# Happy-ZZX/PL-VIWO

Hardware: NVIDIA B200
Metric: front-end frames/sec @1280x560 (higher is better)
Workload: dtype u8/int32 fixed-point + f32 (LK), f64 (sub-pixel, undistort, RANSAC)

## Files before the change

### pl-viwo_b200/csrc/fe_kernels.h

```cpp
#pragma once
#include <cuda_runtime.h>
#include <atomic>
#include <cstdint>

namespace plviwo {

struct SmemOptIn {
  std::atomic<size_t> granted[64];
  SmemOptIn() { for (auto &g : granted) g.store(0); }
  template <class Kernel>
  void ensure(Kernel kernel, size_t bytes) {
    if (bytes <= 48 * 1024) return;
    int dev = 0;
    cudaGetDevice(&dev);
    std::atomic<size_t> &g = granted[dev & 63];
    if (bytes > g.load(std::memory_order_relaxed)) {
      cudaFuncSetAttribute(kernel, cudaFuncAttributeMaxDynamicSharedMemorySize, (int)bytes);
      g.store(bytes, std::memory_order_relaxed);
    }
  }
};

int carveout_percent();
struct CarveoutOnce {
  std::atomic<bool> done[64];
  CarveoutOnce() { for (auto &d : done) d.store(false); }
  template <class Kernel>
  void apply(Kernel kernel) {
    const int pct = carveout_percent();
    if (pct < 0) return;
    int dev = 0;
    cudaGetDevice(&dev);
    std::atomic<bool> &d = done[dev & 63];
    if (d.load(std::memory_order_relaxed)) return;
    cudaFuncSetAttribute(kernel, cudaFuncAttributePreferredSharedMemoryCarveout, pct);
    d.store(true, std::memory_order_relaxed);
  }
};
#define PLVIWO_CARVEOUT(kernel)   \
  do {                            \
    static CarveoutOnce c__;      \
    c__.apply(kernel);            \
  } while (0)

struct DevImage {
  uint8_t *p = nullptr;
  int w = 0, h = 0, pitch = 0;
};

constexpr int kMaxLevels = 8;
constexpr int kFastBandRows = 16;
constexpr int kMaxWin = 31;

struct Pyramid {
  DevImage lvl[kMaxLevels];
  int n = 0;
};

void launch_hist(const DevImage &src, unsigned *d_hist, cudaStream_t s);
void launch_eq_pyr1(const DevImage &src, unsigned *d_hist, unsigned *d_counter, int equalize, const DevImage &l0,
                    const DevImage &l1, const DevImage &half, cudaStream_t s, const uint8_t *d_clahe_luts = nullptr);
void launch_clahe_lut(const DevImage &src, uint8_t *d_luts, cudaStream_t s);
void launch_pyr_rest(const Pyramid &pyr, unsigned *d_counter, cudaStream_t s);
void launch_pyr_down(const DevImage &src, const DevImage &dst, cudaStream_t s);

void launch_signal(int *host_flag, int value, cudaStream_t s);
void launch_signal_inc(int *host_flag, int *dev_seq, cudaStream_t s);
void init_fld_constants();
void init_device_constants();

struct FastCell {
  int x, y, w, h;
};
void launch_fast(const DevImage &img, const FastCell *d_cells, int n_cells, int max_bands, int max_cell_w, int threshold,
                 unsigned *d_total, int *d_band_off, int *d_band_cnt, unsigned *d_kps, int kps_cap, cudaStream_t s);

void launch_fast_select(const FastCell *d_cells, int n_cells, int max_bands, unsigned *d_total, const int *d_band_off,
                        const int *d_band_cnt, const unsigned *d_kps, int kps_cap, unsigned *d_scratch, int nfg,
                        float2 *d_cand_sel, int *d_cand_cnt, cudaStream_t s);
void host_sort_corners(unsigned *v, int n, int keep = 0);

void launch_corner_subpix(const DevImage &img, const float2 *d_in, float2 *d_out, int n, cudaStream_t s,
                          const int *d_cnt = nullptr, int stride = 0);

struct LkParams {
  int win;
  int max_level;
  int max_count;
  float eps_sq;
  float min_eig;
  double K[4], D[4];
  int undistort;
};
bool launch_lk(const Pyramid &prev, const Pyramid &next, const float2 *d_pts0, float2 *d_pts1, uint8_t *d_status,
               float2 *d_p0n, float2 *d_p1n, int n, const LkParams &prm, cudaStream_t s, int *host_flag = nullptr,
               int flag_value = 0, unsigned *d_done_counter = nullptr, const int *d_tab_cnt = nullptr, int tab_stride = 0,
               bool flow_is_zero = false, const unsigned *cell_mask = nullptr);
bool lk_table_mode_ok(const LkParams &prm, int pyramid_images);
void launch_undistort(const float2 *d_pts, float2 *d_out, int n, const double K[4], const double D[4], cudaStream_t s);

struct FldBuffers {
  unsigned *edges = nullptr;
  int words_per_row = 0;
  int *label = nullptr;
  int *cnt = nullptr;
  int *bbox = nullptr;
  int *lroots = nullptr;
  int *lroot_n = nullptr;
  int lroot_cap = 0;
  int *comp_root = nullptr;
  int *counters = nullptr;
  int2 *chain_pts = nullptr;
  int *chain_seed = nullptr, *chain_off = nullptr, *chain_len = nullptr, *order = nullptr;
  int max_chains = 0;
  float4 *segs = nullptr;
  int *seg_cnt = nullptr;
  float4 *out = nullptr;
  int out_cap = 0;
  int alloc(int w, int h, int length_threshold, int out_capacity);
  void release();
};
constexpr int kMaxLineBatch = 8;
struct FldBatch {
  int n = 0;
  DevImage half[kMaxLineBatch];
  FldBuffers f[kMaxLineBatch];
  __host__ __device__ const DevImage &half_of(int k) const { return half[k]; }
  __host__ __device__ const FldBuffers &fld_of(int k) const { return f[k]; }
};
void launch_canny_batch(const FldBatch &b, float th_low, float th_high, cudaStream_t s);
void launch_fld_batch(const FldBatch &b, int length_threshold, float distance_threshold, cudaStream_t s, cudaEvent_t *ev = nullptr);
constexpr int kSegsPerChainDiv = 21;
void launch_canny(const DevImage &half, float th_low, float th_high, FldBuffers &fb, cudaStream_t s);
void launch_fld(const DevImage &half, int length_threshold, float distance_threshold, FldBuffers &fb, cudaStream_t s,
                cudaEvent_t *ev = nullptr);
void launch_unpack_edges(const FldBuffers &fb, int w, int h, uint8_t *d_out, cudaStream_t s);

struct SlotRec {
  DevImage raw;
  DevImage lvl[kMaxLevels];
  int n_lvl;
  DevImage half;
  uint8_t *mask;
  unsigned *hist, *counters;
  uint8_t *clahe;
  unsigned *fast_total;
  unsigned *kps, *sort_scratch;
  int *band_off, *band_cnt;
  float2 *cand, *cand_ref;
  int *cand_cnt;
  FldBuffers fld;
};
struct FrontJob {
  const uint8_t *src;
  int src_pitch;
  int slot;
  int eq_mode;
  int flags;
};
struct FrontGeom {
  int w, h;
  int n_cells, max_bands, max_cell_w, fast_threshold, kps_cap, nfg;
  const FastCell *cells;
};
void launch_hist_batch(const SlotRec *slots, const FrontJob *jobs, int n_jobs, const FrontGeom &g, int *slot_flags, cudaStream_t s);
void launch_clahe_lut_batch(const SlotRec *slots, const FrontJob *jobs, int n_jobs, const FrontGeom &g, cudaStream_t s);
void launch_eq_pyr1_batch(const SlotRec *slots, const FrontJob *jobs, int n_jobs, const FrontGeom &g, bool want_half, cudaStream_t s);
void launch_pyr_level_batch(const SlotRec *slots, const FrontJob *jobs, int n_jobs, int level, int dw, int dh, cudaStream_t s);
void launch_fast_batch(const SlotRec *slots, const FrontJob *jobs, int n_jobs, const FrontGeom &g, cudaStream_t s);
void launch_fast_select_batch(const SlotRec *slots, const FrontJob *jobs, int n_jobs, const FrontGeom &g, cudaStream_t s);
void launch_corner_subpix_batch(const SlotRec *slots, const FrontJob *jobs, int n_jobs, const FrontGeom &g, cudaStream_t s);
struct FldTable {
  const SlotRec *slots;
  const int *idx;
  __device__ const DevImage &half_of(int k) const { return slots[idx[k]].half; }
  __device__ const FldBuffers &fld_of(int k) const { return slots[idx[k]].fld; }
};
void launch_canny_table(const SlotRec *slots, const int *line_slots, int n_jobs, int w, int h, float th_low, cudaStream_t s);
void launch_fld_table(const SlotRec *slots, const int *line_slots, int n_jobs, int w, int h, int max_chains, int length_threshold,
                      float distance_threshold, cudaStream_t s, cudaEvent_t *ev = nullptr);

}
```

### pl-viwo_b200/csrc/kernels_lines.cu

```cuda
#include "fe_kernels.h"

#include <cstdlib>

#include <algorithm>
#include <mutex>
#include <cstdio>
#include <cmath>

namespace plviwo {

__global__ void k_unpack_edges(const unsigned *__restrict__ edges, int words_per_row, int w, int h,
                               uint8_t *__restrict__ out) {
  int x = blockIdx.x * blockDim.x + threadIdx.x, y = blockIdx.y;
  if (x < w && y < h) out[(size_t)y * w + x] = ((edges[(size_t)y * words_per_row + (x >> 5)] >> (x & 31)) & 1u) ? 255 : 0;
}
void launch_unpack_edges(const FldBuffers &fb, int w, int h, uint8_t *d_out, cudaStream_t s) {
  dim3 grid((w + 255) / 256, h);
  PLVIWO_CARVEOUT(k_unpack_edges);
  k_unpack_edges<<<grid, 256, 0, s>>>(fb.edges, fb.words_per_row, w, h, d_out);
}

__device__ __forceinline__ int ccl_find(const int *parent, int i) {
  int p = __ldcg(parent + i);
  while (p != i) {
// ... 155 lines not shown
  const FldBuffers &fb = b.fld_of(blockIdx.z);
  const unsigned *__restrict__ edges = fb.edges;
  const int words_per_row = fb.words_per_row;
  __shared__ CclTileSmem sm;
  const int tid = threadIdx.x;
  const int x0 = blockIdx.x * kTileW, y0 = blockIdx.y * kTileH;
  if (tid < kTileH * 2) {
    const int r = tid >> 1, k = tid & 1;
    const int gy = y0 + r, gw = (x0 >> 5) + k;
    unsigned v = 0;
    if (gy < h && gw < words_per_row) v = edges[(size_t)gy * words_per_row + gw];
    if (gy < h && (gw << 5) + 32 > w) v &= (gw << 5) < w ? (0xffffffffu >> (32 - (w - (gw << 5)))) : 0u;
    sm.bits[r][k] = v;
  }
  __syncthreads();
  ccl_tile_body(fb, sm, x0, y0, w, h);
}

template <class B>
__global__ void k_ccl_reset(const __grid_constant__ B b) {
  const FldBuffers &fb = b.fld_of(blockIdx.x);
  if (threadIdx.x < 12) fb.counters[threadIdx.x] = 0;
  if (threadIdx.x == 12) *fb.lroot_n = 0;
}

constexpr int kCnW = 64, kCnH = 16, kCnThreads = 256;

static_assert(kCnW == kTileW && kCnH == kTileH && kCnThreads == kTileThreads, "Canny tile = connected-component tile");
struct CannySmem {
  uint8_t pix[kCnH + 4][kCnW + 4];
  short sdx[kCnH + 2][kCnW + 2];
  short sdy[kCnH + 2][kCnW + 2];
  unsigned short mag[kCnH + 2][kCnW + 2];
};
template <class B, bool kFuse>
__global__ void __launch_bounds__(kCnThreads)
    k_canny(const __grid_constant__ B b, int low) {
  const uint8_t *__restrict__ img = b.half_of(blockIdx.z).p;
  const int w = b.half_of(blockIdx.z).w, h = b.half_of(blockIdx.z).h, pitch = b.half_of(blockIdx.z).pitch;
  unsigned *__restrict__ edges = b.fld_of(blockIdx.z).edges;
  const int words_per_row = b.fld_of(blockIdx.z).words_per_row;
  __shared__ __align__(16) uint8_t smem_raw[kFuse ? (sizeof(CclTileSmem) > sizeof(CannySmem) ? sizeof(CclTileSmem) : sizeof(CannySmem))
                                                  : sizeof(CannySmem)];
  __shared__ unsigned s_bits[kCnH][2];
  CannySmem &cs = *reinterpret_cast<CannySmem *>(smem_raw);
  auto &pix = cs.pix;
  auto &sdx = cs.sdx;
  auto &sdy = cs.sdy;
  auto &mag = cs.mag;
  const int tx0 = blockIdx.x * kCnW, ty0 = blockIdx.y * kCnH;
  const int tid = threadIdx.x;
  for (int i = tid; i < (kCnH + 4) * (kCnW + 4); i += kCnThreads) {
    int r = i / (kCnW + 4), c = i - r * (kCnW + 4);
    int gx = min(max(tx0 - 2 + c, 0), w - 1), gy = min(max(ty0 - 2 + r, 0), h - 1);
    pix[r][c] = img[(size_t)gy * pitch + gx];
  }
  __syncthreads();
  for (int i = tid; i < (kCnH + 2) * (kCnW + 2); i += kCnThreads) {
    int r = i / (kCnW + 2), c = i - r * (kCnW + 2);
    int gx = tx0 - 1 + c, gy = ty0 - 1 + r;
    int dx = 0, dy = 0, m = 0;
    if (gx >= 0 && gx < w && gy >= 0 && gy < h) {
      const uint8_t *p = &pix[r + 1][c + 1];
      const int s = kCnW + 4;
      dx = (p[-s + 1] + 2 * p[1] + p[s + 1]) - (p[-s - 1] + 2 * p[-1] + p[s - 1]);
      dy = (p[s - 1] + 2 * p[s] + p[s + 1]) - (p[-s - 1] + 2 * p[-s] + p[-s + 1]);
      m = abs(dx) + abs(dy);
    }
    sdx[r][c] = (short)dx;
    sdy[r][c] = (short)dy;
    mag[r][c] = (unsigned short)m;
  }
  __syncthreads();
  const int wv = tid >> 5, lane = tid & 31;
#pragma unroll
  for (int q = 0; q < 4; q++) {
    int r = 2 * wv + (q >> 1), c = (q & 1) * 32 + lane;
    int gx = tx0 + c, gy = ty0 + r;
    bool edge = false;
    if (gx < w && gy < h) {
      int m = mag[r + 1][c + 1];
      if (m > low) {
        int dx = sdx[r + 1][c + 1], dy = sdy[r + 1][c + 1];
        int x = abs(dx), y = abs(dy) << 15;
        int tg22x = x * 13573;
        if (y < tg22x) {
          edge = m > mag[r + 1][c] && m >= mag[r + 1][c + 2];
        } else {
          int tg67x = tg22x + (x << 16);
          if (y > tg67x) {
            edge = m > mag[r][c + 1] && m >= mag[r + 2][c + 1];
          } else {
            int s = (dx ^ dy) < 0 ? -1 : 1;
            edge = m > mag[r][c + 1 - s] && m > mag[r + 2][c + 1 + s];
          }
        }
      }
      if (gy < 6 && gx < 6) edge = false;
      if (gy >= h - 5 && gx >= w - 5) edge = false;
    }
    unsigned bits = __ballot_sync(0xffffffffu, edge);
    if (lane == 0 && gy < h && (tx0 + (q & 1) * 32) < w) edges[(size_t)gy * words_per_row + ((tx0 + (q & 1) * 32) >> 5)] = bits;
    if (kFuse && lane == 0) s_bits[r][q & 1] = bits;
  }
  if (kFuse) {
    __syncthreads();
    CclTileSmem &ts = *reinterpret_cast<CclTileSmem *>(smem_raw);
    if (tid < kCnH * 2) ts.bits[tid >> 1][tid & 1] = s_bits[tid >> 1][tid & 1];
    __syncthreads();
    ccl_tile_body(b.fld_of(blockIdx.z), ts, tx0, ty0, w, h);
  }
}

template <class B>
static void launch_canny_any(const B &b, int n, int w, int h, float th_low, cudaStream_t s, bool fuse_labels = false) {
  dim3 grid((w + kCnW - 1) / kCnW, (h + kCnH - 1) / kCnH, n);
  if (fuse_labels) {
    PLVIWO_CARVEOUT(k_ccl_reset<B>);
    k_ccl_reset<B><<<n, 32, 0, s>>>(b);
    PLVIWO_CARVEOUT((k_canny<B, true>));
    k_canny<B, true><<<grid, kCnThreads, 0, s>>>(b, (int)floorf(th_low));
    return;
  }
  PLVIWO_CARVEOUT((k_canny<B, false>));
  k_canny<B, false><<<grid, kCnThreads, 0, s>>>(b, (int)floorf(th_low));
}
void launch_canny_batch(const FldBatch &b, float th_low, float th_high, cudaStream_t s) {
  (void)th_high;
  launch_canny_any(b, b.n, b.half[0].w, b.half[0].h, th_low, s);
}
void launch_canny_table(const SlotRec *slots, const int *line_slots, int n_jobs, int w, int h, float th_low, cudaStream_t s) {
  if (n_jobs <= 0) return;
  launch_canny_any(FldTable{slots, line_slots}, n_jobs, w, h, th_low, s, true);
}
void launch_canny(const DevImage &half, float th_low, float th_high, FldBuffers &fb, cudaStream_t s) {
  FldBatch b;
  b.n = 1;
  b.half[0] = half;
  b.f[0] = fb;
  launch_canny_batch(b, th_low, th_high, s);
}

template <class B>
__global__ void k_ccl_border(const __grid_constant__ B b, int w, int h) {
  const FldBuffers &fb = b.fld_of(blockIdx.y);
  const unsigned *__restrict__ edges = fb.edges;
  const int words_per_row = fb.words_per_row;
  int *__restrict__ label = fb.label;
  const int nrow = (h - 1) / kTileH, ncol = (w - 1) / kTileW;
  const int t = blockIdx.x * blockDim.x + threadIdx.x;
  if (t < nrow * w) {
    const int y = (t / w + 1) * kTileH, x = t % w;
    if (!edge_at(edges, words_per_row, x, y)) return;
    const int i = y * w + x;
    if (x > 0 && edge_at(edges, words_per_row, x - 1, y - 1)) ccl_union(label, i, i - w - 1);
    if (edge_at(edges, words_per_row, x, y - 1)) ccl_union(label, i, i - w);
    if (x < w - 1 && edge_at(edges, words_per_row, x + 1, y - 1)) ccl_union(label, i, i - w + 1);
    return;
  }
  const int u = t - nrow * w;
  if (u >= ncol * h) return;
  const int x = (u / h + 1) * kTileW, y = u % h;
  if (!edge_at(edges, words_per_row, x, y)) return;
  const int i = y * w + x;
  if (y > 0 && edge_at(edges, words_per_row, x - 1, y - 1)) ccl_union(label, i, i - w - 1);
  if (edge_at(edges, words_per_row, x - 1, y)) ccl_union(label, i, i - 1);
  if (y < h - 1 && edge_at(edges, words_per_row, x - 1, y + 1)) ccl_union(label, i, i + w - 1);
}

template <class B>
__global__ void k_ccl_link(const __grid_constant__ B b, int w, int h) {
  const FldBuffers &fb = b.fld_of(blockIdx.y);
  int *__restrict__ label = fb.label, *__restrict__ cnt = fb.cnt, *__restrict__ bbox = fb.bbox;
  const int nl = min(*fb.lroot_n, fb.lroot_cap);
  const int n = w * h;
  for (int t = blockIdx.x * blockDim.x + threadIdx.x; t < nl; t += gridDim.x * blockDim.x) {
    const int i = fb.lroots[t];
    const int root = ccl_find(label, i);
    if (root == i) continue;
    atomicExch(label + i, root);
    atomicAdd(cnt + root, cnt[i]);
    atomicMax(bbox + root, bbox[i]);
    atomicMin(bbox + n + root, bbox[n + i]);
    atomicMax(bbox + 2 * n + root, bbox[2 * n + i]);
  }
}

constexpr int kPadRows = 2;
constexpr int kWalkThreads = 128;
constexpr int kWalkWarps = kWalkThreads / 32;
constexpr int kSliceWords = 1600;
constexpr int kTMaxW = 62, kTMaxH = 44;
constexpr int kTRows = kTMaxH + 2;
constexpr int kTLanes = 64;
__host__ __device__ inline int comp_cap_big(int n) { return n / 128 + 1; }

template <class B>
__global__ void k_ccl_roots(const __grid_constant__ B b, int w, int h, int min_pixels, int thread_class) {
  const FldBuffers &fb = b.fld_of(blockIdx.y);
  const int *__restrict__ label = fb.label, *__restrict__ cnt = fb.cnt, *__restrict__ bbox = fb.bbox;
  int *__restrict__ comp_root = fb.comp_root, *__restrict__ counters = fb.counters;
  const int max_comps = fb.max_chains;
  const int nl = min(*fb.lroot_n, fb.lroot_cap);
  const int n = w * h;
  for (int t = blockIdx.x * blockDim.x + threadIdx.x; t < nl; t += gridDim.x * blockDim.x) {
    const int i = fb.lroots[t];
    if (label[i] != i) continue;
    const int c = cnt[i];
    if (c < min_pixels) continue;
    const int bh = bbox[i] - i / w + 1;
    const int groups = (bbox[2 * n + i] >> 5) - (bbox[n + i] >> 5) + 1;
    const int bw = bbox[2 * n + i] - bbox[n + i] + 1;
    if (thread_class && bw <= kTMaxW && bh <= kTMaxH) {
      const int q = atomicAdd(counters + 6, 1);
      if (q < max_comps) comp_root[comp_cap_big(n) + max_comps + q] = i;
    } else if ((bh + 2 * kPadRows) * (groups + 2) > kSliceWords) {
      const int q = atomicAdd(counters + 0, 1);
      if (q < comp_cap_big(n)) comp_root[q] = i;
    } else {
      const int q = atomicAdd(counters + 5, 1);
      if (q < max_comps) comp_root[comp_cap_big(n) + q] = i;
    }
  }
}

static int choose_neighbour_host(unsigned mask, int direction) {
  const int i0 = direction < 0 ? direction + 8 : direction;
  if ((mask >> i0) & 1u) return i0;
  const int ia = (i0 + 1) & 7, ib = (i0 + 7) & 7;
  const bool sa = (mask >> ia) & 1u, sb = (mask >> ib) & 1u;
  if (sa && sb) return ia > ib ? ia : ib;
  if (sa) return ia;
  if (sb) return ib;
  return 8;
}
static inline int nb_dr(int i) { return (i <= 2) ? 1 : ((i == 3 || i == 7) ? 0 : -1); }
static inline int nb_dc(int i) { return (i == 0 || i == 6 || i == 7) ? 1 : ((i == 1 || i == 5) ? 0 : -1); }

constexpr int kKeys = 256;
constexpr int kLut1 = 2 * kKeys * 8;
constexpr int kLut2 = 8 * 8 * 8;
constexpr int kLutSize = kLut1 + kLut2;
__device__ __align__(16) uint8_t g_walk_lut[kLutSize];
static bool g_walk_lut_ready[64] = {false};

void init_fld_constants() {
  static std::mutex mu;
  std::lock_guard<std::mutex> lk(mu);
  int dev = 0;
  cudaGetDevice(&dev);
  if (g_walk_lut_ready[dev & 63]) return;
  static uint8_t lut[kLutSize];
  static const int key_bit[8] = {7, 6, 5, 3, 0, 1, 2, 4};
  for (int first = 0; first < 2; first++)
    for (unsigned key = 0; key < (unsigned)kKeys; key++) {
      unsigned mask = 0;
      for (int i = 0; i < 8; i++) mask |= ((key >> key_bit[i]) & 1u) << i;
      for (int d = 0; d < 8; d++) {
        int i = 8;
        if (mask) i = first ? __builtin_ffs((int)mask) - 1 : choose_neighbour_host(mask, d - 3);
        const int dr = i < 8 ? nb_dr(i) : 0, dc = i < 8 ? nb_dc(i) : 0;
        lut[(first * kKeys + key) * 8 + d] = (uint8_t)(i | ((dr + 1) << 4) | ((dc + 1) << 6));
      }
    }
  for (int sc = 0; sc < 8; sc++)
    for (int d = 0; d < 8; d++)
      for (int i = 0; i < 8; i++) {
        const int cd = i > 4 ? i - 8 : i;
        const int nd = sc == 0 ? cd : ((d - 3) * sc + cd) / (sc + 1);
        lut[kLut1 + (sc * 8 + d) * 8 + i] = (uint8_t)(nd + 3);
      }
  cudaMemcpyToSymbol(g_walk_lut, lut, sizeof(lut));
  g_walk_lut_ready[dev & 63] = true;
}

__device__ __forceinline__ unsigned lds_u32(unsigned addr) {
  unsigned v;
  asm volatile("ld.shared.u32 %0, [%1];" : "=r"(v) : "r"(addr) : "memory");
  return v;
}
__device__ __forceinline__ unsigned lds_u8(unsigned addr) {
  unsigned v;
  asm volatile("ld.shared.u8 %0, [%1];" : "=r"(v) : "r"(addr) : "memory");
  return v;
}
__device__ __forceinline__ uint2 lds_u64(unsigned addr) {
  uint2 v;
  asm volatile("ld.shared.v2.u32 {%0, %1}, [%2];" : "=r"(v.x), "=r"(v.y) : "r"(addr) : "memory");
  return v;
}
__device__ __forceinline__ void sts_u32(unsigned addr, unsigned v) {
  asm volatile("st.shared.u32 [%0], %1;" ::"r"(addr), "r"(v) : "memory");
}

struct WalkCtx {
  const unsigned *edges;
  int words_per_row;
  const int *label, *cnt, *bbox;
  int *counters;
  int2 *chain_pts;
  int *chain_seed, *chain_off, *chain_len;
  int max_chains, w, n, length_threshold;
  bool vec4;
};

__device__ __forceinline__ void walk_gather(const WalkCtx &c, unsigned *bm, int root, int y0, int g0, int groups, int bh, int ws,
                                            int wi, int nw, int lane) {
  const int segs = (groups + 3) >> 2;
  const int items = bh * segs;
  const unsigned gmask = 0xffu << (lane & 24);
  for (int it0 = wi * 4; it0 < items; it0 += nw * 4) {
    int4 lab[4];
    unsigned nib[4];
#pragma unroll
    for (int u = 0; u < 4; u++) {
      const int it = it0 + u;
      nib[u] = 0;
      lab[u] = make_int4(-2, -2, -2, -2);
      if (it < items) {
        const int ly = it / segs, sg = it - ly * segs;
        const int g = 4 * sg + (lane >> 3);
        if (g < groups) {
          const unsigned e = __ldg(c.edges + (size_t)(y0 + ly) * c.words_per_row + g0 + g);
          nib[u] = (e >> (4 * (lane & 7))) & 15u;
          if (nib[u]) {
            const int *lp = c.label + (size_t)(y0 + ly) * c.w + ((g0 + g) << 5) + 4 * (lane & 7);
            if (c.vec4) {
              lab[u] = *reinterpret_cast<const int4 *>(lp);
            } else {
              if (nib[u] & 1u) lab[u].x = lp[0];
              if (nib[u] & 2u) lab[u].y = lp[1];
              if (nib[u] & 4u) lab[u].z = lp[2];
              if (nib[u] & 8u) lab[u].w = lp[3];
            }
          }
        }
      }
    }
#pragma unroll
    for (int u = 0; u < 4; u++) {
      const int it = it0 + u;
      const int l4[4] = {lab[u].x, lab[u].y, lab[u].z, lab[u].w};
      unsigned bits = 0;
#pragma unroll
      for (int k = 0; k < 4; k++) {
        if (!((nib[u] >> k) & 1u)) continue;
        int l = l4[k];
        if (l != root) l = __ldg(c.label + l);
        bits |= (l == root ? 1u : 0u) << k;
      }
      bits = (bits & nib[u]) << (4 * (lane & 7));
      const unsigned word = __reduce_or_sync(gmask, bits);
      if ((lane & 7) == 0 && word && it < items) {
        const int ly = it / segs, sg = it - ly * segs;
        bm[(ly + kPadRows) * ws + 1 + 4 * sg + (lane >> 3)] = word;
      }
    }
  }
}

__device__ __forceinline__ void walk_component(const WalkCtx &c, unsigned *bm, unsigned lut_addr, int root, int y0, int g0, int groups,
                                               int bh, int ws, int lane) {
  const int my_dr = lane < 25 ? lane / 5 - 2 : 0;
  const int my_dc = lane < 25 ? lane % 5 - 2 : 0;
  int npts = 0;
  if (lane == 0) npts = atomicAdd(c.counters + 2, c.cnt[root]);
  npts = __shfl_sync(0xffffffffu, npts, 0);
  const int xbase = (g0 << 5) - 32;
  const unsigned bm_addr = (unsigned)__cvta_generic_to_shared(bm);
  const int my_off = my_dr * ws;
  int sy = 0, sg = 0;
  while (sy < bh) {
    const int g = sg + lane;
    const unsigned v = g < groups ? bm[(sy + kPadRows) * ws + 1 + g] : 0u;
    const unsigned any = __ballot_sync(0xffffffffu, v != 0);
    __syncwarp();
    if (!any) {
      sg += 32;
      if (sg >= groups) { sg = 0; sy++; }
      continue;
    }
    const int first = __ffs(any) - 1;
    const unsigned wv = __shfl_sync(0xffffffffu, v, first);
    sg += first;
    int p = ((sg + 1) << 5) + __ffs(wv) - 1, cy = sy;
    int rb = (cy + kPadRows) * ws;
    const int start = npts;
    const int seed = (y0 + cy) * c.w + xbase + p;
    int step = 0;
    unsigned dsel = 0, sh = 6;
    unsigned tb = lut_addr + kKeys * 8;
    if (lane == 0) sts_u32(bm_addr + 4u * (unsigned)(rb + (p >> 5)), wv & ~(1u << (p & 31)));
    __syncwarp();
    unsigned Bw;
    {
      const int qb = p + my_dc;
      const unsigned word = lds_u32(bm_addr + 4u * (unsigned)(rb + my_off + (qb >> 5)));
      Bw = __ballot_sync(0xffffffffu, (word >> (qb & 31)) & 1u);
      __syncwarp();
    }
    while (true) {
      const int qb = p + my_dc;
      const unsigned waddr = bm_addr + 4u * (unsigned)(rb + my_off + (qb >> 5));
      const unsigned word = lds_u32(waddr);
      const unsigned Bs = Bw >> sh;
      const unsigned key = (Bs & 7u) | ((Bs >> 2) & 8u) | ((Bs >> 3) & 16u) | ((Bs >> 5) & 0xE0u);
      const uint2 ev = lds_u64(tb + key * 8u);
      if (lane == 0) c.chain_pts[npts] = make_int2(xbase + p, y0 + cy);
      npts++;
      Bw = __ballot_sync(0xffffffffu, (word >> (qb & 31)) & 1u);
      __syncwarp();
      const unsigned e = __byte_perm(ev.x, ev.y, dsel);
      const unsigned i = e & 15u;
      if (i == 8u) break;
      dsel = lds_u8(lut_addr + kLut1 + ((unsigned)min(step, 7) * 8u + dsel) * 8u + i);
      step++;
      tb = lut_addr;
      const unsigned r1 = (e >> 4) & 3u, c1 = (e >> 6) & 3u;
      sh = 5u * r1 + c1;
      if (lane == (int)(sh + 6u)) sts_u32(waddr, word & ~(1u << (qb & 31)));
      __syncwarp();
      p += (int)c1 - 1;
      cy += (int)r1 - 1;
      rb += ((int)r1 - 1) * ws;
    }
    if (npts - start < c.length_threshold + 1) {
      npts = start;
    } else if (lane == 0) {
      const int k = atomicAdd(c.counters + 3, 1);
      if (k < c.max_chains) {
        c.chain_seed[k] = seed;
        c.chain_off[k] = start;
        c.chain_len[k] = npts - start;
      }
    }
  }
}

__device__ __forceinline__ void walk_component_single(const WalkCtx &c, unsigned *bm, const uint8_t *lut, int root, int y0, int g0,
                                                      int groups, int bh, int ws) {
  int npts = atomicAdd(c.counters + 2, c.cnt[root]);
  const int xbase = (g0 << 5) - 32;
  int sy = 0, sg = 0;
  while (sy < bh) {
    const int rbs = (sy + kPadRows) * ws;
    unsigned wv = 0;
    while (sg < groups && (wv = bm[rbs + 1 + sg]) == 0u) sg++;
    if (sg >= groups) {
      sg = 0;
      sy++;
      continue;
    }
    int p = ((sg + 1) << 5) + __ffs((int)wv) - 1, cy = sy;
    int rb = rbs;
    const int start = npts;
    const int seed = (y0 + cy) * c.w + xbase + p;
    int step = 0;
    unsigned dsel = 0;
    const uint8_t *tb = lut + kKeys * 8;
    bm[rb + (p >> 5)] = wv & ~(1u << (p & 31));
    while (true) {
      c.chain_pts[npts++] = make_int2(xbase + p, y0 + cy);
      const int q = p - 1, wi = q >> 5, sh = q & 31;
      const unsigned *r0 = bm + rb + wi;
      const unsigned t3 = __funnelshift_r(r0[-ws], r0[-ws + 1], sh) & 7u;
      const unsigned c3 = __funnelshift_r(r0[0], r0[1], sh) & 7u;
      const unsigned b3 = __funnelshift_r(r0[ws], r0[ws + 1], sh) & 7u;
      const unsigned key = t3 | ((c3 & 1u) << 3) | ((c3 >> 2) << 4) | (b3 << 5);
      const unsigned e = tb[key * 8u + dsel];
      const unsigned i = e & 15u;
      if (i == 8u) break;
      dsel = lut[kLut1 + ((unsigned)min(step, 7) * 8u + dsel) * 8u + i];
      step++;
      tb = lut;
      const int dr = (int)((e >> 4) & 3u) - 1, dc = (int)((e >> 6) & 3u) - 1;
      p += dc;
      cy += dr;
      rb += dr * ws;
      bm[rb + (p >> 5)] &= ~(1u << (p & 31));
    }
    if (npts - start < c.length_threshold + 1) {
      npts = start;
    } else {
      const int k = atomicAdd(c.counters + 3, 1);
      if (k < c.max_chains) {
        c.chain_seed[k] = seed;
        c.chain_off[k] = start;
        c.chain_len[k] = npts - start;
      }
    }
  }
}

template <class B>
__global__ void __launch_bounds__(kWalkThreads)
    k_fld_walk_cc(const __grid_constant__ B b, int w, int h, int length_threshold, int coop) {
  const FldBuffers &fb = b.fld_of(blockIdx.y);
  WalkCtx c;
  c.edges = fb.edges;
  c.words_per_row = fb.words_per_row;
  c.label = fb.label;
  c.cnt = fb.cnt;
  c.bbox = fb.bbox;
  c.counters = fb.counters;
  c.chain_pts = fb.chain_pts;
  c.chain_seed = fb.chain_seed;
  c.chain_off = fb.chain_off;
  c.chain_len = fb.chain_len;
  c.max_chains = fb.max_chains;
  c.w = w;
  c.n = w * h;
  c.length_threshold = length_threshold;
  c.vec4 = (w & 3) == 0;
  const int *__restrict__ comp_root = fb.comp_root;
  extern __shared__ __align__(16) uint8_t walk_smem[];
  uint8_t *lut = walk_smem;
  unsigned *arena = reinterpret_cast<unsigned *>(walk_smem + kLutSize);
  __shared__ int s_ci;
  const int tid = threadIdx.x, lane = tid & 31, warp = tid >> 5;
  const int n = c.n;
  const int nBig = min(c.counters[0], comp_cap_big(n));
  const int nSmall = min(c.counters[5], c.max_chains);
  if ((int)blockIdx.x >= nBig && (int)blockIdx.x * kWalkWarps >= nSmall) return;
  for (int i = tid; i < kLutSize / 4; i += kWalkThreads)
    reinterpret_cast<unsigned *>(lut)[i] = reinterpret_cast<const unsigned *>(g_walk_lut)[i];
  const unsigned lut_addr = (unsigned)__cvta_generic_to_shared(lut);
  while (true) {
    __syncthreads();
    if (tid == 0) s_ci = nBig > 0 ? atomicAdd(c.counters + 1, 1) : 0x7fffffff;
    __syncthreads();
    const int q = s_ci;
    if (q >= nBig) break;
    const int root = comp_root[q];
    const int y0 = root / w, y1 = c.bbox[root];
    const int g0 = c.bbox[n + root] >> 5, g1 = c.bbox[2 * n + root] >> 5;
    const int groups = g1 - g0 + 1, bh = y1 - y0 + 1, ws = groups + 2;
    for (int i = tid; i < (bh + 2 * kPadRows) * ws; i += kWalkThreads) arena[i] = 0;
    __syncthreads();
    walk_gather(c, arena, root, y0, g0, groups, bh, ws, warp, kWalkWarps, lane);
    __syncthreads();
    if (warp == 0) {
      if (coop) walk_component(c, arena, lut_addr, root, y0, g0, groups, bh, ws, lane);
      else if (lane == 0) walk_component_single(c, arena, lut, root, y0, g0, groups, bh, ws);
    }
  }
  unsigned *bm = arena + warp * kSliceWords;
  while (true) {
    int q = 0;
    if (lane == 0) q = atomicAdd(c.counters + 7, 1);
    q = __shfl_sync(0xffffffffu, q, 0);
    if (q >= nSmall) break;
    const int root = comp_root[comp_cap_big(n) + q];
    const int y0 = root / w, y1 = c.bbox[root];
    const int g0 = c.bbox[n + root] >> 5, g1 = c.bbox[2 * n + root] >> 5;
    const int groups = g1 - g0 + 1, bh = y1 - y0 + 1, ws = groups + 2;
    for (int i = lane; i < (bh + 2 * kPadRows) * ws; i += 32) bm[i] = 0;
    __syncwarp();
    walk_gather(c, bm, root, y0, g0, groups, bh, ws, 0, 1, lane);
    __syncwarp();
    if (coop) walk_component(c, bm, lut_addr, root, y0, g0, groups, bh, ws, lane);
    else if (lane == 0) walk_component_single(c, bm, lut, root, y0, g0, groups, bh, ws);
    __syncwarp();
  }
}

template <class B>
__global__ void __launch_bounds__(kTLanes)
    k_fld_walk_thread(const __grid_constant__ B b, int w, int h, int length_threshold) {
  const FldBuffers &fb = b.fld_of(blockIdx.y);
  const unsigned *__restrict__ edges = fb.edges;
  const int words_per_row = fb.words_per_row;
  const int *__restrict__ label = fb.label, *__restrict__ cnt = fb.cnt, *__restrict__ bbox = fb.bbox;
  int *__restrict__ counters = fb.counters;
  int2 *__restrict__ chain_pts = fb.chain_pts;
  const int max_chains = fb.max_chains;
  const int n = w * h;
  __shared__ __align__(16) uint8_t lut[kLutSize];
  __shared__ unsigned long long bm[kTRows * kTLanes];
  const int tid = threadIdx.x;
  const int nT = min(counters[6], max_chains);
  if ((int)blockIdx.x * kTLanes >= nT) return;
  for (int i = tid; i < kLutSize / 4; i += kTLanes) reinterpret_cast<unsigned *>(lut)[i] = reinterpret_cast<const unsigned *>(g_walk_lut)[i];
  __syncthreads();
  const int *__restrict__ queue = fb.comp_root + comp_cap_big(n) + max_chains;
  unsigned long long *row = bm + tid;
  while (true) {
    const int q = atomicAdd(counters + 8, 1);
    if (q >= nT) break;
    const int root = queue[q];
    const int y0 = root / w, y1 = bbox[root], xmin = bbox[n + root], xmax = bbox[2 * n + root];
    const int bh = y1 - y0 + 1, bw = xmax - xmin + 1;
    row[0] = 0ull;
    row[(bh + 1) * kTLanes] = 0ull;
    const int w0 = xmin >> 5, sh = xmin & 31;
    const unsigned long long wmask = (bw >= 64 ? ~0ull : ((1ull << bw) - 1ull));
    for (int r = 0; r < bh; r++) {
      const unsigned *er = edges + (size_t)(y0 + r) * words_per_row;
      const unsigned e0 = er[w0], e1 = w0 + 1 < words_per_row ? er[w0 + 1] : 0u, e2 = w0 + 2 < words_per_row ? er[w0 + 2] : 0u;
      unsigned long long v = ((unsigned long long)e0 | ((unsigned long long)e1 << 32)) >> sh;
      if (sh) v |= (unsigned long long)e2 << (64 - sh);
      v &= wmask;
      unsigned long long mine = 0ull;
      const int base = (y0 + r) * w + xmin;
      while (v) {
        const int bpos = __ffsll((long long)v) - 1;
        v &= v - 1;
        int l = label[base + bpos];
        if (l != root) l = label[l];
        if (l == root) mine |= 1ull << bpos;
      }
      row[(r + 1) * kTLanes] = mine << 1;
    }
    int npts = atomicAdd(counters + 2, cnt[root]);
    const int xorg = xmin - 1, yorg = y0 - 1;
    int sy = 1;
    bool in_chain = false;
    int cy = 0, cx = 0, start = 0, seed = 0, step = 0;
    unsigned dsel = 0;
    const uint8_t *tb = lut;
    while (true) {
      if (!in_chain) {
        if (sy > bh) break;
        const unsigned long long R = row[sy * kTLanes];
        if (R == 0ull) {
          sy++;
          continue;
        }
        cx = __ffsll((long long)R) - 1;
        cy = sy;
        row[sy * kTLanes] = R & ~(1ull << cx);
        start = npts;
        seed = (yorg + cy) * w + xorg + cx;
        step = 0;
        dsel = 0;
        tb = lut + kKeys * 8;
        in_chain = true;
      }
      chain_pts[npts++] = make_int2(xorg + cx, yorg + cy);
      const unsigned long long Ra = row[(cy - 1) * kTLanes], Rc = row[cy * kTLanes], Rb = row[(cy + 1) * kTLanes];
      const unsigned t3 = (unsigned)(Ra >> (cx - 1)) & 7u, c3 = (unsigned)(Rc >> (cx - 1)) & 7u, b3 = (unsigned)(Rb >> (cx - 1)) & 7u;
      const unsigned key = t3 | ((c3 & 1u) << 3) | ((c3 >> 2) << 4) | (b3 << 5);
      const unsigned e = tb[key * 8u + dsel];
      const unsigned i = e & 15u;
      if (i == 8u) {
        if (npts - start < length_threshold + 1) {
          npts = start;
        } else {
          const int k = atomicAdd(counters + 3, 1);
          if (k < max_chains) {
            fb.chain_seed[k] = seed;
            fb.chain_off[k] = start;
            fb.chain_len[k] = npts - start;
          }
        }
        in_chain = false;
        continue;
      }
      dsel = lut[kLut1 + ((unsigned)min(step, 7) * 8u + dsel) * 8u + i];
      step++;
      tb = lut;
      const int dr = (int)((e >> 4) & 3u) - 1, dc = (int)((e >> 6) & 3u) - 1;
      cy += dr;
      cx += dc;
      const unsigned long long Rn = dr < 0 ? Ra : (dr > 0 ? Rb : Rc);
      row[cy * kTLanes] = Rn & ~(1ull << cx);
    }
  }
}

template <class B>
__global__ void k_fld_order(const __grid_constant__ B b) {
  const FldBuffers &fb = b.fld_of(blockIdx.y);
  const int *__restrict__ chain_seed = fb.chain_seed, *__restrict__ counters = fb.counters;
  int *__restrict__ order = fb.order;
  const int max_chains = fb.max_chains;
  const int n = min(counters[3], max_chains);
  const int c = blockIdx.x * blockDim.x + threadIdx.x;
  if (c >= n) return;
  const int mine = chain_seed[c];
  int rank = 0;
  for (int k = 0; k < n; k++) rank += chain_seed[k] < mine ? 1 : 0;
  order[rank] = c;
}

struct FitSums {
  double x, y, x2, y2, xy;
  int n;
};
__device__ __forceinline__ void fs_add(FitSums &s, int2 p) {
  float px = (float)p.x, py = (float)p.y;
  s.x += px; s.y += py;
  s.x2 += px * px; s.y2 += py * py; s.xy += px * py;
  s.n++;
}
__device__ __forceinline__ void fs_line(const FitSums &s, double l[3]) {
  double w = (float)s.n;
  double x = s.x / w, y = s.y / w, x2 = s.x2 / w, y2 = s.y2 / w, xy = s.xy / w;
  double dx2 = x2 - x * x, dy2 = y2 - y * y, dxy = xy - x * y;
  float t = (float)atan2(2 * dxy, dx2 - dy2) / 2;
  float l0 = cosf(t), l1 = sinf(t), l2 = (float)x, l3 = (float)y;
  double a[3] = {l2, l3, 1.0};
  double b[3] = {(double)(l2 + l0), (double)(l3 + l1), 1.0};
  l[0] = a[1] * b[2] - a[2] * b[1];
  l[1] = a[2] * b[0] - a[0] * b[2];
  l[2] = a[0] * b[1] - a[1] * b[0];
}
__device__ __forceinline__ double dist_point_line(double px, double py, double l[3]) {
  double x = l[0], y = l[1];
  double n2 = x * x + y * y;
  if (n2 != 1.0) {
    double w = sqrt(n2);
    l[0] = x / w; l[1] = y / w; l[2] = l[2] / w;
  }
  return l[0] * px + l[1] * py + l[2];
}
__device__ __forceinline__ void incident_point(const double l[3], float &px, float &py, int W, int H) {
  double a[3] = {(double)px, (double)py, 1.0};
  double b[3] = {l[0], l[1], 0.0};
  double lk[3] = {a[1] * b[2] - a[2] * b[1], a[2] * b[0] - a[0] * b[2], a[0] * b[1] - a[1] * b[0]};
  double xk[3] = {lk[1] * l[2] - lk[2] * l[1], lk[2] * l[0] - lk[0] * l[2], lk[0] * l[1] - lk[1] * l[0]};
  double alpha = 1.0 / xk[2];
  float fx = (float)(xk[0] * alpha), fy = (float)(xk[1] * alpha);
  px = fx < 0.0f ? 0.0f : (fx >= (W - 1.0f) ? (W - 1.0f) : fx);
  py = fy < 0.0f ? 0.0f : (fy >= (H - 1.0f) ? (H - 1.0f) : fy);
}

template <class B>
__global__ void k_fld_segments(const __grid_constant__ B b, int T, float dist_thr) {
  const FldBuffers &fb = b.fld_of(blockIdx.y);
  const uint8_t *__restrict__ img = b.half_of(blockIdx.y).p;
  const int W = b.half_of(blockIdx.y).w, H = b.half_of(blockIdx.y).h, pitch = b.half_of(blockIdx.y).pitch;
  const int2 *__restrict__ chain_pts = fb.chain_pts;
  const int *__restrict__ chain_off = fb.chain_off, *__restrict__ chain_len = fb.chain_len, *__restrict__ order = fb.order;
  const int *__restrict__ counters = fb.counters;
  const int max_chains = fb.max_chains;
  float4 *__restrict__ segs = fb.segs;
  int *__restrict__ seg_cnt = fb.seg_cnt, *__restrict__ seg_base = fb.seg_cnt + fb.max_chains;
  const int r = blockIdx.x * blockDim.x + threadIdx.x;
  if (r >= min(counters[3], max_chains)) return;
  const int c = order[r];
  const int2 *points = chain_pts + chain_off[c];
  const int total = chain_len[c];
  const int slot0 = chain_off[c] / kSegsPerChainDiv;
  int nseg = 0;
  int i, j;
  for (i = 0; i + T < total; i++) {
    int2 ps = points[i], pe = points[i + T];
    double l[3] = {(double)ps.y - (double)pe.y, (double)pe.x - (double)ps.x,
                   (double)ps.x * (double)pe.y - (double)ps.y * (double)pe.x};
    bool is_line = true;
    FitSums fs = {0, 0, 0, 0, 0, 0};
    fs_add(fs, ps);
    for (j = 1; j < T; j++) {
      int2 pt = points[i + j];
      double dist = dist_point_line((double)pt.x, (double)pt.y, l);
      if (fabs(dist) > dist_thr) { is_line = false; break; }
      fs_add(fs, pt);
    }
    if (!is_line) continue;
    fs_add(fs, pe);
    fs_line(fs, l);
    {
      float fx = (float)ps.x, fy = (float)ps.y;
      incident_point(l, fx, fy, W, H);
      ps.x = __float2int_rn(fx);
      ps.y = __float2int_rn(fy);
    }
    for (j = T + 1; i + j < total; j++) {
      int2 pt = points[i + j];
      double dist = dist_point_line((double)pt.x, (double)pt.y, l);
      if (fabs(dist) > dist_thr) {
        fs_line(fs, l);
        dist = dist_point_line((double)pt.x, (double)pt.y, l);
        if (fabs(dist) > dist_thr) { j--; break; }
      }
      pe = pt;
      fs_add(fs, pt);
    }
    fs_line(fs, l);
    float e1x = (float)ps.x, e1y = (float)ps.y, e2x = (float)pe.x, e2y = (float)pe.y;
    incident_point(l, e1x, e1y, W, H);
    incident_point(l, e2x, e2y, W, H);
    i = i + j;
    float len = sqrtf((e1x - e2x) * (e1x - e2x) + (e1y - e2y) * (e1y - e2y));
    if (len < (float)T) continue;
    if ((e1x <= 5.0f && e2x <= 5.0f) || (e1y <= 5.0f && e2y <= 5.0f) || (e1x >= W - 5.0f && e2x >= W - 5.0f) ||
        (e1y >= H - 5.0f && e2y >= H - 5.0f))
      continue;
    if (!(e1x == 0.0f && e2x == 0.0f && e1y == 0.0f && e2y == 0.0f)) {
      double ang = atan2((double)(e2y - e1y), (double)(e2x - e1x));
      double dx = (double)e2x - (double)e1x, dy = (double)e2y - (double)e1y;
      const double kPi = 3.1415926535897932384626433832795;
      double cs = cos(90.0 * kPi / 180.0 + ang), sn = sin(90.0 * kPi / 180.0 + ang);
      int iR = 0, iL = 0;
      for (int k = 0; k < 10; k++) {
        float qx, qy;
        if (k == 0) { qx = e1x; qy = e1y; }
        else if (k == 9) { qx = e2x; qy = e2y; }
        else {
          qx = e1x + ((float)dx / 9.0f * (float)k);
          qy = e1y + ((float)dy / 9.0f * (float)k);
        }
        int rx = __double2int_rn(qx + cs), ry = __double2int_rn(qy + sn);
        int lx = __double2int_rn(qx - cs), ly = __double2int_rn(qy - sn);
        rx = min(max(rx, 0), W - 1); ry = min(max(ry, 0), H - 1);
        lx = min(max(lx, 0), W - 1); ly = min(max(ly, 0), H - 1);
        iR += img[(size_t)ry * pitch + rx];
        iL += img[(size_t)ly * pitch + lx];
      }
      if (iR > iL) {
        float tx = e1x, ty = e1y;
        e1x = e2x; e1y = e2y; e2x = tx; e2y = ty;
      }
    }
    segs[slot0 + nseg] = make_float4(e1x, e1y, e2x, e2y);
    nseg++;
  }
  seg_cnt[r] = nseg;
  seg_base[r] = slot0;
}

template <class B>
__global__ void __launch_bounds__(256)
    k_fld_compact(const __grid_constant__ B b) {
  const FldBuffers &fb = b.fld_of(blockIdx.y);
  const float4 *__restrict__ segs = fb.segs;
  const int *__restrict__ seg_cnt = fb.seg_cnt, *__restrict__ seg_base = fb.seg_cnt + fb.max_chains;
  int *__restrict__ counters = fb.counters;
  const int max_chains = fb.max_chains, out_cap = fb.out_cap;
  float4 *__restrict__ out = fb.out;
  __shared__ int warp_tot[8];
  __shared__ int s_running;
  const int n = min(counters[3], max_chains);
  const int tid = threadIdx.x;
  if (tid == 0) s_running = 0;
  __syncthreads();
  for (int base = 0; base < n; base += 256) {
    int c = base + tid;
    int cnt = c < n ? seg_cnt[c] : 0;
    int v = cnt;
#pragma unroll
    for (int d = 1; d < 32; d <<= 1) {
      int t = __shfl_up_sync(0xffffffffu, v, d);
      if ((tid & 31) >= d) v += t;
    }
    if ((tid & 31) == 31) warp_tot[tid >> 5] = v;
    __syncthreads();
    int off = s_running;
    for (int k = 0; k < (tid >> 5); k++) off += warp_tot[k];
    off += v - cnt;
    for (int k = 0; k < cnt; k++)
      if (off + k < out_cap) out[off + k] = segs[seg_base[c] + k];
    __syncthreads();
    if (tid == 255) s_running = off + cnt;
    __syncthreads();
  }
  if (tid == 0) counters[4] = s_running;
}

int FldBuffers::alloc(int w, int h, int length_threshold, int out_capacity) {
  const size_t n = (size_t)w * h;
  words_per_row = (w + 31) / 32;
  max_chains = (int)(n / (length_threshold + 1)) + 1;
  out_cap = out_capacity;
  bool ok = true;
  auto A = [&](auto **p, size_t bytes) { ok = ok && cudaMalloc((void **)p, bytes) == cudaSuccess; };
  A(&edges, (size_t)words_per_row * h * sizeof(unsigned));
  A(&label, (n + 32) * sizeof(int));
  A(&cnt, n * sizeof(int));
  A(&bbox, 3 * n * sizeof(int));
  A(&comp_root, (size_t)(2 * max_chains + comp_cap_big((int)n)) * sizeof(int));
  A(&counters, 12 * sizeof(int));
  lroot_cap = (int)(n / 4 + 1);
  A(&lroots, (size_t)lroot_cap * sizeof(int));
  A(&lroot_n, sizeof(int));
  A(&chain_pts, n * sizeof(int2));
  A(&chain_seed, (size_t)max_chains * sizeof(int));
  A(&chain_off, (size_t)max_chains * sizeof(int));
  A(&chain_len, (size_t)max_chains * sizeof(int));
  A(&order, (size_t)max_chains * sizeof(int));
  A(&segs, (n / kSegsPerChainDiv + 2) * sizeof(float4));
  A(&seg_cnt, (size_t)2 * max_chains * sizeof(int));
  A(&out, (size_t)out_cap * sizeof(float4));
  if (ok) ok = cudaMemset(counters, 0, 12 * sizeof(int)) == cudaSuccess;
  return ok ? 0 : 1;
}

void FldBuffers::release() {
  cudaFree(lroots); cudaFree(lroot_n);
  cudaFree(edges); cudaFree(label); cudaFree(cnt); cudaFree(bbox); cudaFree(comp_root); cudaFree(counters);
  cudaFree(chain_pts); cudaFree(chain_seed); cudaFree(chain_off); cudaFree(chain_len); cudaFree(order);
  cudaFree(segs); cudaFree(seg_cnt); cudaFree(out);
  *this = FldBuffers();
}

template <class B>
static void launch_fld_any(const B &b, int nb_frames, int w, int h, int max_chains, int length_threshold, float distance_threshold,
                           cudaStream_t s, cudaEvent_t *ev, bool tiles_done = false) {
  const int n = w * h;
  const int tpb = 256;
  const int lroot_cap = n / 4 + 1;
  if (!tiles_done) {
    PLVIWO_CARVEOUT(k_ccl_reset<B>);
    k_ccl_reset<B><<<nb_frames, 32, 0, s>>>(b);
    PLVIWO_CARVEOUT(k_ccl_tile<B>);
    k_ccl_tile<B><<<dim3((w + kTileW - 1) / kTileW, (h + kTileH - 1) / kTileH, nb_frames), kTileThreads, 0, s>>>(b, w, h);
  }
  const int nborder = ((h - 1) / kTileH) * w + ((w - 1) / kTileW) * h;
  if (nborder > 0) {
    PLVIWO_CARVEOUT(k_ccl_border<B>);
    k_ccl_border<B><<<dim3((nborder + tpb - 1) / tpb, nb_frames), tpb, 0, s>>>(b, w, h);
  }
  const int root_ctas = std::max(1, std::min((lroot_cap + tpb - 1) / tpb, 12));
  PLVIWO_CARVEOUT(k_ccl_link<B>);
  k_ccl_link<B><<<dim3(root_ctas, nb_frames), tpb, 0, s>>>(b, w, h);
  PLVIWO_CARVEOUT(k_ccl_roots<B>);
  const char *tmin_env = std::getenv("PLVIWO_WALK_THREAD_MIN");
  const int thread_class = nb_frames >= (tmin_env ? std::max(1, std::atoi(tmin_env)) : 16) ? 1 : 0;
  k_ccl_roots<B><<<dim3(root_ctas, nb_frames), tpb, 0, s>>>(b, w, h, length_threshold + 1, thread_class);
  if (ev) cudaEventRecord(ev[0], s);
  init_fld_constants();
  const int ws = ((w + 31) >> 5) + 2;
  const size_t arena_words = std::max<size_t>((size_t)(h + 2 * kPadRows) * ws, (size_t)kWalkWarps * kSliceWords);
  size_t smem = (size_t)kLutSize + arena_words * sizeof(unsigned);
  static SmemOptIn optin;
  optin.ensure(k_fld_walk_cc<B>, smem);
  static const int walk_ctas_env = [] {
    const char *e = std::getenv("PLVIWO_WALK_CTAS");
    return e ? std::atoi(e) : 0;
  }();
  const int walk_ctas = walk_ctas_env > 0 ? walk_ctas_env : (nb_frames > 1 ? std::max(2, std::min(74, 256 / nb_frames)) : 148);
  const int walk_t = 4;
  if (thread_class) {
    PLVIWO_CARVEOUT(k_fld_walk_thread<B>);
    k_fld_walk_thread<B><<<dim3(walk_t, nb_frames), kTLanes, 0, s>>>(b, w, h, length_threshold);
  }
  PLVIWO_CARVEOUT(k_fld_walk_cc<B>);
  static const int coop = [] { const char *e = std::getenv("PLVIWO_WALK_SINGLE"); return (e && std::atoi(e)) ? 0 : 1; }();
  k_fld_walk_cc<B><<<dim3(walk_ctas, nb_frames), kWalkThreads, smem, s>>>(b, w, h, length_threshold, coop);
  if (ev) cudaEventRecord(ev[1], s);
  PLVIWO_CARVEOUT(k_fld_order<B>);
  k_fld_order<B><<<dim3((max_chains + 127) / 128, nb_frames), 128, 0, s>>>(b);
  PLVIWO_CARVEOUT(k_fld_segments<B>);
  k_fld_segments<B><<<dim3((max_chains + 63) / 64, nb_frames), 64, 0, s>>>(b, length_threshold, distance_threshold);
  PLVIWO_CARVEOUT(k_fld_compact<B>);
  k_fld_compact<B><<<dim3(1, nb_frames), 256, 0, s>>>(b);
}
void launch_fld_batch(const FldBatch &b, int length_threshold, float distance_threshold, cudaStream_t s, cudaEvent_t *ev) {
  launch_fld_any(b, b.n, b.half[0].w, b.half[0].h, b.f[0].max_chains, length_threshold, distance_threshold, s, ev);
}
void launch_fld_table(const SlotRec *slots, const int *line_slots, int n_jobs, int w, int h, int max_chains, int length_threshold,
                      float distance_threshold, cudaStream_t s, cudaEvent_t *ev) {
  if (n_jobs <= 0) return;
  launch_fld_any(FldTable{slots, line_slots}, n_jobs, w, h, max_chains, length_threshold, distance_threshold, s, ev, true);
}

void launch_fld(const DevImage &half, int length_threshold, float distance_threshold, FldBuffers &fb, cudaStream_t s,
                cudaEvent_t *ev) {
  FldBatch b;
  b.n = 1;
  b.half[0] = half;
  b.f[0] = fb;
  launch_fld_batch(b, length_threshold, distance_threshold, s, ev);
}

}
```

Before: 55280.

## Walk small line components per thread over a shared whole-frame edge map

The small-component walk in k_fld_walk_cc is reorganised. Each block now claims a chunk of components and loads the padded edge bitmap of the whole half-resolution frame into shared memory once. Each warp then gathers a sparse list of (word index, root-owned bit mask) pairs for one component into a new global walk_mask buffer. After that, one thread per component traces its chains directly on the shared frame map, using atomic clears. This replaces the per-warp zero, gather and walk into private slices, cutting per-component setup and sync overhead. The cost is an extra n*uint2 buffer, a dependence on counters[2] for offsets, atomics in shared memory, and a whole-frame map that must fit in the arena. The launch bounds also add a minimum of 8 blocks per SM.

```diff
diff --git a/pl-viwo_b200/csrc/fe_kernels.h b/pl-viwo_b200/csrc/fe_kernels.h
--- a/pl-viwo_b200/csrc/fe_kernels.h
+++ b/pl-viwo_b200/csrc/fe_kernels.h
@@ -109,6 +109,7 @@
   int *lroot_n = nullptr;
   int lroot_cap = 0;
   int *comp_root = nullptr;
+  uint2 *walk_mask = nullptr;
   int *counters = nullptr;
   int2 *chain_pts = nullptr;
   int *chain_seed = nullptr, *chain_off = nullptr, *chain_len = nullptr, *order = nullptr;
diff --git a/pl-viwo_b200/csrc/kernels_lines.cu b/pl-viwo_b200/csrc/kernels_lines.cu
--- a/pl-viwo_b200/csrc/kernels_lines.cu
+++ b/pl-viwo_b200/csrc/kernels_lines.cu
@@ -481,6 +481,7 @@
   int *chain_seed, *chain_off, *chain_len;
   int max_chains, w, n, length_threshold;
   bool vec4;
+  uint2 *walk_mask;
 };
 
 __device__ __forceinline__ void walk_gather(const WalkCtx &c, unsigned *bm, int root, int y0, int g0, int groups, int bh, int ws,
@@ -671,8 +672,143 @@
   }
 }
 
+constexpr int kGatherUnroll = 4;
+constexpr int kSeedBatch = 4;
+
+__device__ __forceinline__ int walk_mask_gather(const unsigned *map, int ws, const int *__restrict__ label, int w, bool vec4,
+                                                int root, int y0, int g0, int groups, int bh, uint2 *__restrict__ out, int lane) {
+  const int segs = (groups + 3) >> 2;
+  const int items = bh * segs;
+  const unsigned gmask = 0xffu << (lane & 24);
+  const unsigned lt = (1u << lane) - 1u;
+  int len = 0;
+  for (int it0 = 0; it0 < items; it0 += kGatherUnroll) {
+    int4 lab[kGatherUnroll];
+    unsigned nib[kGatherUnroll], widx[kGatherUnroll];
+#pragma unroll
+    for (int u = 0; u < kGatherUnroll; u++) {
+      const int it = it0 + u;
+      nib[u] = 0;
+      widx[u] = 0;
+      lab[u] = make_int4(-2, -2, -2, -2);
+      if (it < items) {
+        const int ly = it / segs, sg = it - ly * segs;
+        const int g = 4 * sg + (lane >> 3);
+        if (g < groups) {
+          widx[u] = (unsigned)((y0 + ly + 1) * ws + 1 + g0 + g);
+          nib[u] = (map[widx[u]] >> (4 * (lane & 7))) & 15u;
+          if (nib[u]) {
+            const int *lp = label + (size_t)(y0 + ly) * w + ((g0 + g) << 5) + 4 * (lane & 7);
+            if (vec4) {
+              lab[u] = *reinterpret_cast<const int4 *>(lp);
+            } else {
+              if (nib[u] & 1u) lab[u].x = lp[0];
+              if (nib[u] & 2u) lab[u].y = lp[1];
+              if (nib[u] & 4u) lab[u].z = lp[2];
+              if (nib[u] & 8u) lab[u].w = lp[3];
+            }
+          }
+        }
+      }
+    }
+#pragma unroll
+    for (int u = 0; u < kGatherUnroll; u++) {
+      const int l4[4] = {lab[u].x, lab[u].y, lab[u].z, lab[u].w};
+      unsigned bits = 0;
+#pragma unroll
+      for (int k = 0; k < 4; k++) {
+        if (!((nib[u] >> k) & 1u)) continue;
+        int l = l4[k];
+        if (l != root) l = __ldg(label + l);
+        bits |= (l == root ? 1u : 0u) << k;
+      }
+      const unsigned word = __reduce_or_sync(gmask, bits << (4 * (lane & 7)));
+      const bool put = (lane & 7) == 0 && word != 0u;
+      const unsigned bal = __ballot_sync(0xffffffffu, put);
+      if (put) out[len + __popc(bal & lt)] = make_uint2(widx[u], word);
+      len += __popc(bal);
+    }
+  }
+  return len;
+}
+
+__device__ __forceinline__ void walk_frame_component(volatile unsigned *map, int ws, const uint8_t *lut,
+                                                     const uint2 *__restrict__ list, int len, int npts, const WalkCtx &c) {
+  uint2 cur[kSeedBatch], nxt[kSeedBatch];
+#pragma unroll
+  for (int k = 0; k < kSeedBatch; k++) {
+    cur[k] = k < len ? list[k] : make_uint2(0u, 0u);
+    nxt[k] = kSeedBatch + k < len ? list[kSeedBatch + k] : make_uint2(0u, 0u);
+  }
+  int e = 0, k0 = 0;
+  while (true) {
+    unsigned v = 0u, widx = 0u;
+    bool found = false;
+#pragma unroll
+    for (int k = 0; k < kSeedBatch; k++) {
+      const unsigned vk = cur[k].y & map[cur[k].x];
+      if (!found && k >= k0 && vk) {
+        found = true;
+        k0 = k;
+        v = vk;
+        widx = cur[k].x;
+      }
+    }
+    if (!found) {
+      e += kSeedBatch;
+      if (e >= len) break;
+#pragma unroll
+      for (int k = 0; k < kSeedBatch; k++) {
+        cur[k] = nxt[k];
+        nxt[k] = e + kSeedBatch + k < len ? list[e + kSeedBatch + k] : make_uint2(0u, 0u);
+      }
+      k0 = 0;
+      continue;
+    }
+    const int my = (int)widx / ws;
+    int rb = my * ws, cy = my - 1;
+    int p = (((int)widx - rb) << 5) + __ffs((int)v) - 1;
+    const int start = npts;
+    const int seed = cy * c.w + p - 32;
+    int step = 0;
+    unsigned dsel = 0;
+    const uint8_t *tb = lut + kKeys * 8;
+    atomicAnd((unsigned *)&map[rb + (p >> 5)], ~(1u << (p & 31)));
+    while (true) {
+      c.chain_pts[npts++] = make_int2(p - 32, cy);
+      const int q = p - 1, wi = q >> 5, sh = q & 31;
+      volatile unsigned *r0 = map + rb + wi;
+      const unsigned t3 = __funnelshift_r(r0[-ws], r0[-ws + 1], sh) & 7u;
+      const unsigned c3 = __funnelshift_r(r0[0], r0[1], sh) & 7u;
+      const unsigned b3 = __funnelshift_r(r0[ws], r0[ws + 1], sh) & 7u;
+      const unsigned key = t3 | ((c3 & 1u) << 3) | ((c3 >> 2) << 4) | (b3 << 5);
+      const unsigned e8 = tb[key * 8u + dsel];
+      const unsigned i = e8 & 15u;
+      if (i == 8u) break;
+      dsel = lut[kLut1 + ((unsigned)min(step, 7) * 8u + dsel) * 8u + i];
+      step++;
+      tb = lut;
+      const int dr = (int)((e8 >> 4) & 3u) - 1, dc = (int)((e8 >> 6) & 3u) - 1;
+      p += dc;
+      cy += dr;
+      rb += dr * ws;
+      atomicAnd((unsigned *)&map[rb + (p >> 5)], ~(1u << (p & 31)));
+    }
+    if (npts - start < c.length_threshold + 1) {
+      npts = start;
+    } else {
+      const int k = atomicAdd(c.counters + 3, 1);
+      if (k < c.max_chains) {
+        c.chain_seed[k] = seed;
+        c.chain_off[k] = start;
+        c.chain_len[k] = npts - start;
+      }
+    }
+  }
+}
+
 template <class B>
-__global__ void __launch_bounds__(kWalkThreads)
+__global__ void __launch_bounds__(kWalkThreads, 8)
     k_fld_walk_cc(const __grid_constant__ B b, int w, int h, int length_threshold, int coop) {
   const FldBuffers &fb = b.fld_of(blockIdx.y);
   WalkCtx c;
@@ -691,16 +827,18 @@
   c.n = w * h;
   c.length_threshold = length_threshold;
   c.vec4 = (w & 3) == 0;
+  c.walk_mask = fb.walk_mask;
   const int *__restrict__ comp_root = fb.comp_root;
   extern __shared__ __align__(16) uint8_t walk_smem[];
   uint8_t *lut = walk_smem;
   unsigned *arena = reinterpret_cast<unsigned *>(walk_smem + kLutSize);
   __shared__ int s_ci;
+  __shared__ int2 s_span[32];
   const int tid = threadIdx.x, lane = tid & 31, warp = tid >> 5;
   const int n = c.n;
   const int nBig = min(c.counters[0], comp_cap_big(n));
   const int nSmall = min(c.counters[5], c.max_chains);
-  if ((int)blockIdx.x >= nBig && (int)blockIdx.x * kWalkWarps >= nSmall) return;
+  if ((int)blockIdx.x >= nBig && (int)blockIdx.x >= nSmall) return;
   for (int i = tid; i < kLutSize / 4; i += kWalkThreads)
     reinterpret_cast<unsigned *>(lut)[i] = reinterpret_cast<const unsigned *>(g_walk_lut)[i];
   const unsigned lut_addr = (unsigned)__cvta_generic_to_shared(lut);
@@ -723,23 +861,43 @@
       else if (lane == 0) walk_component_single(c, arena, lut, root, y0, g0, groups, bh, ws);
     }
   }
-  unsigned *bm = arena + warp * kSliceWords;
+  if (nSmall == 0) return;
+  const int chunk = min(32, max(1, (nSmall + (int)gridDim.x - 1) / (int)gridDim.x));
+  const int wpr = c.words_per_row, fws = wpr + 2;
+  bool map_ready = false;
   while (true) {
-    int q = 0;
-    if (lane == 0) q = atomicAdd(c.counters + 7, 1);
-    q = __shfl_sync(0xffffffffu, q, 0);
-    if (q >= nSmall) break;
-    const int root = comp_root[comp_cap_big(n) + q];
-    const int y0 = root / w, y1 = c.bbox[root];
-    const int g0 = c.bbox[n + root] >> 5, g1 = c.bbox[2 * n + root] >> 5;
-    const int groups = g1 - g0 + 1, bh = y1 - y0 + 1, ws = groups + 2;
-    for (int i = lane; i < (bh + 2 * kPadRows) * ws; i += 32) bm[i] = 0;
-    __syncwarp();
-    walk_gather(c, bm, root, y0, g0, groups, bh, ws, 0, 1, lane);
-    __syncwarp();
-    if (coop) walk_component(c, bm, lut_addr, root, y0, g0, groups, bh, ws, lane);
-    else if (lane == 0) walk_component_single(c, bm, lut, root, y0, g0, groups, bh, ws);
-    __syncwarp();
+    __syncthreads();
+    if (tid == 0) s_ci = atomicAdd(c.counters + 7, chunk);
+    __syncthreads();
+    const int base = s_ci;
+    if (base >= nSmall) break;
+    const int m = min(chunk, nSmall - base);
+    if (!map_ready) {
+      for (int i = tid; i < (h + 2) * fws; i += kWalkThreads) {
+        const int r = i / fws, k = i - r * fws;
+        unsigned v = 0u;
+        if (r >= 1 && r <= h && k >= 1 && k <= wpr) {
+          const int gw = k - 1;
+          v = c.edges[(size_t)(r - 1) * wpr + gw];
+          if ((gw << 5) + 32 > w) v &= 0xffffffffu >> (32 - (w - (gw << 5)));
+        }
+        arena[i] = v;
+      }
+      __syncthreads();
+      map_ready = true;
+    }
+    for (int j = warp; j < m; j += kWalkWarps) {
+      const int root = comp_root[comp_cap_big(n) + base + j];
+      int off = 0;
+      if (lane == 0) off = atomicAdd(c.counters + 2, c.cnt[root]);
+      off = __shfl_sync(0xffffffffu, off, 0);
+      const int y0 = root / w, g0 = c.bbox[n + root] >> 5;
+      const int len = walk_mask_gather(arena, fws, c.label, w, c.vec4, root, y0, g0, (c.bbox[2 * n + root] >> 5) - g0 + 1,
+                                       c.bbox[root] - y0 + 1, c.walk_mask + off, lane);
+      if (lane == 0) s_span[j] = make_int2(off, len);
+    }
+    __syncthreads();
+    if (tid < m) walk_frame_component(arena, fws, lut, c.walk_mask + s_span[tid].x, s_span[tid].y, s_span[tid].x, c);
   }
 }
 
@@ -1049,6 +1207,7 @@
   A(&cnt, n * sizeof(int));
   A(&bbox, 3 * n * sizeof(int));
   A(&comp_root, (size_t)(2 * max_chains + comp_cap_big((int)n)) * sizeof(int));
+  A(&walk_mask, n * sizeof(uint2));
   A(&counters, 12 * sizeof(int));
   lroot_cap = (int)(n / 4 + 1);
   A(&lroots, (size_t)lroot_cap * sizeof(int));
@@ -1067,7 +1226,7 @@
 
 void FldBuffers::release() {
   cudaFree(lroots); cudaFree(lroot_n);
-  cudaFree(edges); cudaFree(label); cudaFree(cnt); cudaFree(bbox); cudaFree(comp_root); cudaFree(counters);
+  cudaFree(edges); cudaFree(label); cudaFree(cnt); cudaFree(bbox); cudaFree(comp_root); cudaFree(walk_mask); cudaFree(counters);
   cudaFree(chain_pts); cudaFree(chain_seed); cudaFree(chain_off); cudaFree(chain_len); cudaFree(order);
   cudaFree(segs); cudaFree(seg_cnt); cudaFree(out);
   *this = FldBuffers();
```

Measured after the change: 53450, median of 6. -3.3%, worse.
